# Linux-cpp-lisp/navigation-by-deja-vu

Hardware: AMD Instinct MI355X
Metric: view-comparisons/sec (sensor x library x headings) (higher is better)
Workload: dtype u8

## Files before the change

### include/dejavu.h

```cpp
#ifndef DEJAVU_H
#define DEJAVU_H

#include <stdint.h>

#ifdef __cplusplus
extern "C" {
#endif

typedef struct dv_ctx dv_ctx;

enum {
    DV_OK = 0,
    DV_ERR_INVALID = -1,
    DV_ERR_HIP = -2,
    DV_ERR_STATE = -3,
    DV_ERR_OOM = -4,
    DV_ERR_INDEX = -5
};

#define DV_MAX_HEADINGS 64
#define DV_MAX_HUE_PLANES 4

#define DV_STEP_FORCE_RESOLVE 1u
#define DV_STEP_WANT_SCENE    2u
// ... 201 lines not shown
int dv_timer_start(dv_ctx *ctx);
int dv_timer_stop(dv_ctx *ctx, float *elapsed_ms);
int dv_profile_kernel(dv_ctx *ctx, int enable);
int dv_profile_read(dv_ctx *ctx, double *total_ms, int64_t *n_launches);
int dv_workgroup_shape(dv_ctx *ctx, int n_headings, int *shape);
int dv_stream_read_gbps(dv_ctx *ctx, int64_t n_bytes, int iters, double *gbps);

int dv_range_push(const char *name);
int dv_range_pop(void);

int dv_patches_on_level(dv_ctx *ctx);

#define DV_FORM_MATRIX_CORES 1
#define DV_FORM_FP4 2
#define DV_FORM_FUSED_FINISH 4
int dv_scoring_form(dv_ctx *ctx);

const char *dv_version(void);

#ifdef __cplusplus
}
#endif
#endif
```

### navigation-by-deja-vu_amd/csrc/dejavu_hip.hip

```cpp
#include "dejavu_kernels.h"
#include "../../include/dejavu.h"

#include <algorithm>
#include <atomic>
#include <chrono>
#include <cmath>
#include <limits>
#include <cstdarg>
#include <cstddef>
#include <cstdint>
#include <cstdio>
#include <cstdlib>
#include <cstring>
#include <new>
#include <string>
#include <vector>

using namespace dv;

static_assert(sizeof(StepResultDev) == sizeof(dv_step_result) + sizeof(unsigned long long) &&
              offsetof(StepResultDev, check) == sizeof(dv_step_result), "device record = host record + check word");
static_assert(kMaxHeadings == DV_MAX_HEADINGS && kMaxHues == DV_MAX_HUE_PLANES, "header constants differ");
static_assert(kResSenseError == DV_RES_SENSE_ERROR, "header constants differ");

// ... 109 lines not shown
    size_t btile_bytes = 0;
    uint4* d_coef = nullptr;
    bool coef_ready = false;
    bool prep_dwords_ready = false;
    int bits_env = 1;
    int mfma_tiles_env = 0, mfma_chunk_env = 0;
    const int* int_hsconst = nullptr;
    const int* int_vconst = nullptr;
    bool fuse_request = false;
    bool epilogue_fused = false;
    bool fp4_ok = false;
    int fp4_env = 1;
    uint4* d_coef4 = nullptr;
    uint4* d_ctiles = nullptr;
    size_t ctile_bytes = 0;
    int vcode_env = 0;
    int last_form = 0;
    int fuse_env = 1;
    int lc_env = 1;
    int ht_env = 2;
    int ring_env = 0;
    int mixed_env = 1;
    int tune_all_env = 0;
    int fail_alloc_env = 0;
    int lib_allocs = 0;
    int fused_nb = 0;
    int group_pad_kb = -1;
    int allow_signed = 1;
    double* d_fam = nullptr;
    double* d_scene = nullptr;
    StepState* d_state = nullptr;
// ... 111 lines not shown
static void use_set(dv_ctx* c, int which);
static void diffuse_free(dv_ctx* c);
static void free_library(dv_ctx* c) {
    auto F = [](auto*& p) { if (p) { (void)hipFree(p); p = nullptr; } };
    use_set(c, 0);
    for (int j = 0; j < dv_ctx::kExtraSets; ++j) {
        dv_ctx::PassSet& a = c->extra[j];
        F(a.raw); F(a.coef); F(a.coef4); F(a.acc); F(a.bsum); F(a.ctmp); F(a.state); F(a.cand); F(a.cand_exact);
        a = dv_ctx::PassSet{};
    }
    c->n_extra = 0;
    F(c->d_tiles); F(c->d_raw_patches); F(c->d_prep); F(c->d_acc); F(c->d_one); F(c->d_fam); F(c->d_scene);
    F(c->d_part); F(c->d_pmax); F(c->d_record); F(c->d_keys); F(c->d_bsum); F(c->d_bsum2); F(c->d_ctmp);
    F(c->d_ftiles); F(c->d_fraw); F(c->d_fprep); F(c->d_fpart); F(c->d_fprep4); F(c->d_fvnorm); F(c->d_fpnorm); F(c->d_flower); F(c->d_fprepb);
    F(c->d_u8tiles); F(c->d_u8raw); F(c->d_u8prep); F(c->d_u8part); F(c->d_vnorm); F(c->d_pnorm);
    F(c->d_btiles); F(c->d_coef); F(c->d_coef4); F(c->d_ctiles); c->ctile_bytes = 0;
    c->pbits = PrepBits{};
    c->bits_ok = false; c->coef_ready = false; c->btile_bytes = 0;
    c->metric = 0;
    F(c->d_state); F(c->d_cand); F(c->d_cand_exact);
    if (c->h_result) { (void)hipHostFree(c->h_result); c->h_result = nullptr; c->d_result = nullptr; }
    if (c->h_scene) { (void)hipHostFree(c->h_scene); c->h_scene = nullptr; }
    F(c->d_scene_b);
    if (c->h_scene_b) { (void)hipHostFree(c->h_scene_b); c->h_scene_b = nullptr; }
    c->scene_b_cap = 0;
    c->have_lib = false;
    for (int i = 0; i < 4; ++i) c->tuned_shape[i] = 0;
    c->A = 0;
    c->step_pending = false;
}

// ... 208 lines not shown
    return DV_OK;
}

extern "C" int dv_synchronize(dv_ctx* c) {
    if (!c) return DV_ERR_INVALID;
    HIP_TRY(c, hipSetDevice(c->device));
    HIP_TRY(c, hipStreamSynchronize(c->stream));
    return DV_OK;
}

static long long group_stride(const dv_ctx* c, long long kb) {
    const long long pad = c->group_pad_kb >= 0 ? c->group_pad_kb : ((kb & 1) ? 0 : 1);
    return (kb + pad) * 64;
}

static int build_bit_planes(dv_ctx* c) {
    const LibCfg& g = c->cfg;
    c->bits_ok = false;
    c->fp4_ok = false;
    c->mixed = false;
    if (c->bits_env == 0 || c->metric != 0 || g.generic) return DV_OK;
    unsigned* d_presence = nullptr;
    uint32_t presence[(kMaxHues + 1) * 8];
    HIP_TRY(c, hipMalloc(&d_presence, sizeof presence));
    hipError_t e = hipMemsetAsync(d_presence, 0, sizeof presence, c->stream);
    if (e == hipSuccess) {
        hipLaunchKernelGGL(k_level_scan, dim3(2048), dim3(256), 0, c->stream, c->d_tiles, c->cfg, d_presence);
        e = hipGetLastError();
    }
    if (e == hipSuccess) e = hipMemcpyAsync(presence, d_presence, sizeof presence, hipMemcpyDeviceToHost, c->stream);
// ... 64 lines not shown
    for (int k = 0; k < kMaxBitPlanes; ++k)
        pb.tbl[k] = (unsigned)b.pl[k] | ((unsigned)b.lo[k] << 8) | ((unsigned)b.w[k] << 16) | ((unsigned)b.wfull[k] << 24);
    HIP_TRY(c, hipMemsetAsync(c->d_coef, 0, (size_t)2 * nkt * 8192, c->stream));
    if (c->fp4_ok) HIP_TRY(c, hipMemsetAsync(c->d_coef4, 0, (size_t)2 * nkt * 4096, c->stream));
    for (int bp = 0; bp < g.npl; ++bp) {
        pb.lmin[bp] = b.lmin[bp];
        for (int v = 0; v < 256; ++v) {
            const bool level = (presence[bp * 8 + (v >> 5)] >> (v & 31)) & 1u;
            if ((mixed && bp < g.nhs) || level || v <= (int)b.lmin[bp] || v >= (int)b.lmax[bp]) pb.ok[bp][v >> 5] |= 1u << (v & 31);
        }
    }
    c->pbits = pb;
    c->mixed = mixed;
    b.vcode = 0;
    b.GSC = b.GS;
    if (c->fp4_ok && five_levels) {
        const long long units = 4ll * b.NK[0] + 3ll * b.NK[1];
        long long kib = (units + 3) / 4;
        if (kib % 2 == 0) ++kib;
        b.GSC = (int)(kib * 4);
        if (hipMalloc(&c->d_ctiles, (size_t)G32 * b.GSC * 256) == hipSuccess) {
            b.vcode = 1;
            c->ctile_bytes = (size_t)G32 * units * 256;
        } else {
            (void)hipGetLastError();
            b.GSC = b.GS;
        }
    }
    b.nt = c->nt_env >= 0 ? c->nt_env : 1;
    c->bcfg = b;
    const long long total_t = G32 * nkt * 64;
    hipLaunchKernelGGL(k_bitpack, dim3((unsigned)((total_t + 255) / 256)), dim3(256), 0, c->stream, c->d_tiles, c->d_btiles, c->cfg, b);
    HIP_TRY(c, hipGetLastError());
    if (b.vcode) {
        hipLaunchKernelGGL(k_bitpack_code, dim3((unsigned)((total_t + 255) / 256)), dim3(256), 0, c->stream, c->d_btiles,
                           reinterpret_cast<unsigned*>(c->d_ctiles), c->cfg, b);
        HIP_TRY(c, hipGetLastError());
    }
    HIP_TRY(c, hipStreamSynchronize(c->stream));
    c->bits_ok = true;
    c->coef_ready = false;
    return DV_OK;
}

static const unsigned* offlevel_word(const dv_ctx* c) {
    return c->fp4_ok ? &c->d_acc[c->acc_parity].off : c->d_one;
}
static int enqueue_bit_prep(dv_ctx* c, bool force = false) {
    (void)force;
// ... 1101 lines not shown
    return word == 0 ? 1 : 0;
}

extern "C" int dv_patches_on_level(dv_ctx* c) {
    if (!c) return DV_ERR_INVALID;
    if (!c->have_lib || !c->bits_ok || !c->fp4_ok) return fail(c, DV_ERR_STATE, "this library has no fp4 form");
    if (!c->coef_ready) return fail(c, DV_ERR_STATE, "no coefficient image of the resident patches yet");
    return read_on_level(c);
}

extern "C" int dv_scoring_form(dv_ctx* c) {
    if (!c) return DV_ERR_INVALID;
    if (!(c->last_form & DV_FORM_FP4)) return c->last_form;
    const int on_level = read_on_level(c);
    if (on_level < 0) return on_level;
    return on_level ? c->last_form : c->last_form & ~DV_FORM_FP4;
}

extern "C" int dv_clear_library(dv_ctx* c) {
    if (!c) return DV_ERR_INVALID;
    HIP_TRY(c, hipSetDevice(c->device));
    HIP_TRY(c, hipStreamSynchronize(c->stream));
    free_library(c);
    return DV_OK;
}

extern "C" int dv_get_library_info(const dv_ctx* c, dv_lib_info* o) {
    if (!c || !o) return DV_ERR_INVALID;
    if (!c->have_lib) return DV_ERR_STATE;
    memset(o, 0, sizeof *o);
    o->n_views = c->cfg.F;
// ... 6 lines not shown
    o->signed_saturation = c->cfg.signed_s;
    o->has_value_plane = c->cfg.hasv;
    o->tile_bytes = (int64_t)c->tile_bytes;
    o->chem_weight = c->cfg.cw;
    o->delta = c->delta;
    for (int k = 0; k < kMaxHues; ++k) o->hues[k] = c->cfg.hues[k];
    o->n_hues = 0;
    if (c->cfg.has_hs && !c->cfg.generic) o->n_hues = c->cfg.signed_s ? 2 : c->cfg.nhs;
    o->weight_lo = c->cfg.hasv ? 0.0 : 1.0;
    o->weight_hi = c->cfg.has_hs ? 1.0 : 0.0;
    o->has_bit_planes = c->bits_ok ? 1 : 0;
    o->fp4_form = (c->bits_ok && c->fp4_ok) ? 1 : 0;
    o->bit_planes_hs = c->bits_ok ? c->bcfg.T[0] : 0;
    o->bit_planes_v = c->bits_ok ? c->bcfg.T[1] : 0;
    o->bit_tile_bytes = c->bits_ok ? (int64_t)c->btile_bytes : 0;
    o->code_tile_bytes = (c->bits_ok && c->bcfg.vcode) ? (int64_t)c->ctile_bytes : 0;
    o->mixed_layout = (c->bits_ok && c->mixed) ? 1 : 0;
    return DV_OK;
}

extern "C" int dv_read_planes(dv_ctx* c, int64_t v0, int64_t n, uint8_t* out) {
    if (!c || !out) return DV_ERR_INVALID;
    if (!c->have_lib) return fail(c, DV_ERR_STATE, "no library set");
    if (v0 < 0 || n < 1 || v0 + n > c->cfg.F) return fail(c, DV_ERR_INVALID, "view range [%lld, %lld) outside the library", (long long)v0, (long long)(v0 + n));
    HIP_TRY(c, hipSetDevice(c->device));
    const long long total = n * c->cfg.npl * (long long)c->cfg.P;
    unsigned char* d = nullptr;
    HIP_TRY(c, hipMalloc(&d, (size_t)total));
    hipLaunchKernelGGL(k_read_planes, dim3((unsigned)((total + 255) / 256)), dim3(256), 0, c->stream, c->d_tiles, d, c->cfg,
                       (long long)v0, (long long)n);
    hipError_t e = hipGetLastError();
// ... 158 lines not shown

static FuseArgs fuse_args(const dv_ctx* c) {
    FuseArgs fz{};
    fz.wts = wts_ptr(c);
    fz.hsconst = c->d_acc[c->acc_parity].bhs;
    fz.vconst = c->d_acc[c->acc_parity].bv;
    fz.bsum = c->d_bsum;
    fz.ctmp = c->d_ctmp;
    fz.st = c->d_state;
    fz.A_real = c->A;
    fz.A_agent = c->A_agent;
    fz.delta = c->delta;
    return fz;
}

enum class Body { Ring, Ring2, RingA, RingB, Lc, LcShort, LcCode, LcReg, Lc2Tiles, Lc2TilesCode, Lc22, Count };

struct BodyShape { int SK8, RD8, SK4, RD4, TILES, SKL, RDL; bool LCODE; int HT; };
constexpr BodyShape kBodyShapes[] = {
     {4, 2, 2, 4, 1, 0, 3, false, 1},
     {1, 3, 2, 3, 2, 0, 3, false, 1},
     {4, 2, 2, 6, 1, 0, 3, false, 1},
     {4, 2, 4, 3, 1, 0, 3, false, 1},
     {4, 2, 2, 4, 1, 4, 3, false, 1},
     {4, 2, 2, 4, 1, 2, 5, false, 1},
     {4, 2, 2, 4, 1, 4, 3, true, 1},
     {4, 2, 2, 4, 1, kLregStage, 3, false, 1},
     {4, 2, 2, 4, 1, 4, 3, false, 2},
     {4, 2, 2, 4, 1, 4, 3, true, 2},
     {4, 2, 0, 0, 1, 2, 3, false, 2},
};
static_assert(sizeof kBodyShapes / sizeof kBodyShapes[0] == (size_t)Body::Count, "one shape per body");
constexpr BodyShape body_shape(Body b) { return kBodyShapes[(int)b]; }

template <Body B, bool FUSE>
constexpr auto body_kernel() {
    constexpr BodyShape s = body_shape(B);
    if constexpr (B == Body::Lc22) return &k_sad_lc22<s.SKL, s.RDL>;
    else return &k_sad_mfma_dual<s.SK8, s.RD8, s.SK4, s.RD4, s.TILES, FUSE, s.SKL, s.RDL, s.LCODE, s.HT>;
}

constexpr int body_view_groups(Body b) { return b == Body::Lc22 ? 8 : 8 * body_shape(b).TILES / body_shape(b).HT; }
// ... 17 lines not shown

template <Body B, bool FUSE>
static void launch_body(dv_ctx* c, int nchunk, int has_hs) {
    constexpr BodyShape s = body_shape(B);
    constexpr int lds = body_lds_bytes<B, FUSE>();
    static_assert(body_lds_bytes<B, true>() <= 160 * 1024, "LDS");
    constexpr auto kernel = body_kernel<B, FUSE>();
    static const hipError_t attr_set = hipFuncSetAttribute((const void*)kernel, hipFuncAttributeMaxDynamicSharedMemorySize, lds);
    (void)attr_set;
    const long long n_gq = item_groups(c->cfg.Fpad / 32, body_view_groups(B));
    const long long items = n_gq * nchunk;
    const unsigned grid = (unsigned)(items < 256 ? items : 256);
    const int nkt = c->bcfg.NK[0] + c->bcfg.NK[1];
    FuseArgs fz{};
    if (FUSE) { fz = fuse_args(c); fz.nb = (int)grid; }
    for (int a_off = 0; a_off < c->APAD; a_off += 32 * s.HT) {
        const uint4* coef = c->d_coef + (size_t)(a_off / 32) * nkt * 512;
        const uint4* coef4 = c->fp4_ok ? c->d_coef4 + (size_t)(a_off / 32) * nkt * 256 : nullptr;
        if constexpr (B == Body::Lc22) {
            hipLaunchKernelGGL(kernel, dim3(grid), dim3(512), lds, c->stream, c->d_btiles, coef, coef4, offlevel_word(c), c->cfg, c->bcfg,
                               c->APAD, a_off, has_hs, fz, (int)n_gq);
        } else {
            hipLaunchKernelGGL(kernel, dim3(grid), dim3(512), lds, c->stream, c->d_btiles, c->bcfg.vcode ? c->d_ctiles : c->d_btiles, coef,
                               coef4, offlevel_word(c), reinterpret_cast<int*>(c->d_part), c->cfg, c->bcfg, nchunk, c->APAD, a_off, has_hs,
                               fz, (int)n_gq);
        }
    }
    if (FUSE) { c->epilogue_fused = true; c->fused_nb = (int)grid; }
}

static bool shared_accumulator_fits(const dv_ctx* c, bool with_bit0) {
    if (!c->fp4_ok || c->bcfg.vcode || c->mixed) return false;
    for (int seg = 0; seg < 2; ++seg) {
        int w = 0;
        for (int bit = 1; bit < 4; ++bit) {
            const int wb = c->bcfg.wacc[seg][bit];
            if (wb && w && wb != w) return false;
            if (wb) w = wb;
        }
        if (with_bit0 && seg == 0 && c->bcfg.wacc[0][0] && w && c->bcfg.wacc[0][0] != w) return false;
    }
    return true;
}
static bool lc22_fits(const dv_ctx* c) {
    return shared_accumulator_fits(c, true) && (long long)c->bcfg.NK[0] * 256 <= 32767;
}
static bool lreg_fits(const dv_ctx* c) {
    return shared_accumulator_fits(c, false) && c->bcfg.NK[0] % kLregStage == 0;
}

struct MfmaPlan { Body body; int nchunk; bool fuses; };
static MfmaPlan mfma_plan(dv_ctx* c, int apad, bool fuse_request) {
    const long long G32 = c->cfg.Fpad / 32;
    const bool may_fuse = fuse_request && c->fuse_env && !c->mfma_chunk_env;
    const bool use_lc = c->lc_env != 0 && c->fp4_ok && !c->mfma_tiles_env;
    Body body;
    if (use_lc) {
        const bool two_tiles = apad == 64 && c->ht_env == 2;
        if (two_tiles && may_fuse && c->lc22_env && lc22_fits(c) && item_groups(G32, 8) >= 160) body = Body::Lc22;
        else if (two_tiles) body = c->bcfg.vcode ? Body::Lc2TilesCode : Body::Lc2Tiles;
        else if (c->bcfg.vcode) body = Body::LcCode;
        else body = c->lc_env == 2 ? Body::LcShort : Body::Lc;
    } else {
        const int tiles = c->mfma_tiles_env ? c->mfma_tiles_env : (G32 >= 16ll * 320 ? 2 : 1);
        body = tiles == 2 ? Body::Ring2 : (c->ring_env == 1 ? Body::RingA : (c->ring_env == 2 ? Body::RingB : Body::Ring));
        if (body == Body::Ring2 && !c->mfma_tiles_env) {
            static const bool spills[2] = {kernel_uses_scratch((const void*)body_kernel<Body::Ring2, false>()),
                                           kernel_uses_scratch((const void*)body_kernel<Body::Ring2, true>())};
            const bool will_fuse = may_fuse && item_groups(G32, body_view_groups(Body::Ring2)) >= 160;
            if (spills[will_fuse ? 1 : 0]) body = c->ring_env == 1 ? Body::RingA : (c->ring_env == 2 ? Body::RingB : Body::Ring);
        }
    }
    const long long GQ = item_groups(G32, body_view_groups(body));
    int nchunk = 1;
    if (c->mfma_chunk_env) {
        nchunk = c->mfma_chunk_env;
    } else if (GQ < 160) {
        nchunk = (int)((256 + GQ - 1) / GQ);
    }
    const int nk_min = c->bcfg.NK[1] > 0 ? (c->bcfg.NK[0] > 0 && c->bcfg.NK[0] < c->bcfg.NK[1] ? c->bcfg.NK[0] : c->bcfg.NK[1]) : c->bcfg.NK[0];
    while (nchunk > 1 && nk_min / nchunk < 4) --nchunk;
    if (nchunk > c->nchunk_cap) nchunk = c->nchunk_cap;
    if (nchunk < 1 || c->mixed) nchunk = 1;
    if (body == Body::Lc && nchunk == 1 && c->lreg_env && lreg_fits(c)) body = Body::LcReg;
    return {body, nchunk, fuse_request && c->fuse_env && nchunk == 1};
}

static bool batch_pass_fuses(dv_ctx* c, int apad) {
    if (c->metric != 0 || c->exact || c->cfg.generic || !c->bits_ok || c->mixed) return false;
    const int cls = apad_class(apad);
    const int shape = c->shape_env ? c->shape_env : c->tuned_shape[cls];
    if (shape != 6) return false;
    return mfma_plan(c, apad, true).fuses;
}

template <Body B>
static void launch_planned(dv_ctx* c, const MfmaPlan& p, int has_hs) {
    if constexpr (B != Body::Lc22) {
        if (!p.fuses) return launch_body<B, false>(c, p.nchunk, has_hs);
    }
    launch_body<B, true>(c, p.nchunk, has_hs);
}

static void launch_mfma(dv_ctx* c, int has_hs) {
    const MfmaPlan p = mfma_plan(c, c->APAD, c->fuse_request);
    c->nchunk = p.nchunk;
    switch (p.body) {
        case Body::Ring: return launch_planned<Body::Ring>(c, p, has_hs);
        case Body::Ring2: return launch_planned<Body::Ring2>(c, p, has_hs);
        case Body::RingA: return launch_planned<Body::RingA>(c, p, has_hs);
        case Body::RingB: return launch_planned<Body::RingB>(c, p, has_hs);
        case Body::Lc: return launch_planned<Body::Lc>(c, p, has_hs);
        case Body::LcShort: return launch_planned<Body::LcShort>(c, p, has_hs);
        case Body::LcCode: return launch_planned<Body::LcCode>(c, p, has_hs);
        case Body::LcReg: return launch_planned<Body::LcReg>(c, p, has_hs);
        case Body::Lc2Tiles: return launch_planned<Body::Lc2Tiles>(c, p, has_hs);
        case Body::Lc2TilesCode: return launch_planned<Body::Lc2TilesCode>(c, p, has_hs);
        case Body::Lc22: return launch_planned<Body::Lc22>(c, p, has_hs);
        case Body::Count: break;
    }
}

static int launch_int_scoring(dv_ctx* c, hipEvent_t after_tiles, int* n_partial, bool with_combine = true) {
    const LibCfg& g = c->cfg;
    int has_hs_sum, has_v_sum = g.hasv;
    c->int_hsconst = c->d_acc[c->acc_parity].hs;
    c->int_vconst = nullptr;
    c->epilogue_fused = false;
    c->last_form = 0;
    if (needs_prep_dwords(c)) { const int rc = ensure_prep_dwords(c); if (rc) return rc; }
// ... 6 lines not shown
            HIP_TRY(c, hipGetLastError());
            c->hs_bytes_pass = true;
            const int keep = c->force_shape;
            c->force_shape = c->APAD >= 16 ? 2 : 1;
            switch (g.nhs) {
                case 1: launch_tiles_apad<1, 0>(c); break;
                case 2: launch_tiles_apad<2, 0>(c); break;
                case 3: launch_tiles_apad<3, 0>(c); break;
                default: launch_tiles_apad<4, 0>(c); break;
            }
            c->force_shape = keep;
            c->hs_bytes_pass = false;
            c->nchunk = 1;
        } else
        launch_mfma(c, has_hs_sum);
        c->last_form = DV_FORM_MATRIX_CORES | (c->fp4_ok ? DV_FORM_FP4 : 0) | (c->epilogue_fused ? DV_FORM_FUSED_FINISH : 0);
        c->int_hsconst = c->mixed ? c->d_acc[c->acc_parity].hs : c->d_acc[c->acc_parity].bhs;
        c->int_vconst = c->d_acc[c->acc_parity].bv;
    } else if (g.generic) {
        has_hs_sum = 1;
        if (g.hasv) launch_generic_apad<1, 1>(c); else launch_generic_apad<1, 0>(c);
    } else {
        has_hs_sum = g.nhs > 0 ? 1 : 0;
        switch (g.nhs * 2 + g.hasv) {
            case 1: launch_tiles_apad<0, 1>(c); break;
            case 2: launch_tiles_apad<1, 0>(c); break;
            case 3: launch_tiles_apad<1, 1>(c); break;
            case 4: launch_tiles_apad<2, 0>(c); break;
            case 5: launch_tiles_apad<2, 1>(c); break;
            case 6: launch_tiles_apad<3, 0>(c); break;
            case 7: launch_tiles_apad<3, 1>(c); break;
// ... 998 lines not shown
```

### navigation-by-deja-vu_amd/csrc/dejavu_kernels.h

```cpp
#pragma once
#include <hip/hip_runtime.h>
#include <stdint.h>
#include <type_traits>

#pragma clang fp contract(off)

namespace dv {

#ifdef DEJAVU_STAMPS
#ifdef DEJAVU_EXP_FIN
#define DV_EXP_FIN_ON 1
#else
#define DV_EXP_FIN_ON 0
#endif
__device__ unsigned long long g_dv_stamps[256 * 8];
#define DV_STAMP(i) do { if (threadIdx.x == 0) { g_dv_stamps[(blockIdx.x & 255) * 8 + (i)] = __builtin_amdgcn_s_memrealtime(); \
    if (((i) == 1 || (i) == 2) && !DV_EXP_FIN_ON) g_dv_stamps[(blockIdx.x & 255) * 8 + 5 + (i)] = __builtin_amdgcn_s_memtime(); } } while (0)
#else
#define DV_STAMP(i) do { } while (0)
#endif

constexpr int kMaxHeadings = 64;
constexpr int kMaxHues = 4;
constexpr int kCandCap = 4096;
// ... 3609 lines not shown
        }
    }
    }
    if constexpr (FUSE) {
#pragma unroll
        for (int h = 0; h < HT; ++h)
            if (a_off + 32 * h < fz.A_real) fused_block_end(scratch0 + h * 64, fz, c, a_off + 32 * h);
    }
    DV_STAMP(5);
}

constexpr int kLregStage = 8;
template <int SK, int RD>
constexpr int lreg_ring_bytes() { return RD * SK * 4 * 1024; }

template <int SK, int RD, bool FUSE>
__device__ __forceinline__ void
sad_lc_fp4_lreg(const uint4* __restrict__ btiles, const uint4* __restrict__ coef4, int* __restrict__ part, const LibCfg& c, const BitCfg& b,
                int apad_total, int a_off, int has_hs_sum, const FuseArgs& fz, int n_gq) {
    extern __shared__ uint4 lds_ring[];
    constexpr int TL = 2;
    constexpr int NW = 8, NC = 4;
    constexpr int KCOEF = 4;
    constexpr int SLOTB = SK * KCOEF * 1024;
    constexpr int PER = SK;
    constexpr int RING = RD * SLOTB;
    static_assert(PER * (RD - 1) < 64 && SK % 2 == 0 && RD >= 3, "ring shape");
    const int lane = threadIdx.x & 63;
    const int wave = __builtin_amdgcn_readfirstlane(threadIdx.x >> 6);
    const bool loader = wave >= NC;
    const long long G32 = c.Fpad / 32, GQ = n_gq;
    const int NKT = b.NK[0] + b.NK[1];
    const int nst = (NKT + SK - 1) / SK;
    const int NK0 = b.NK[0];
    const long long gbytes = (long long)b.GS * 1024;
    const unsigned lds_base = (unsigned)(unsigned long long)(lds_ptr_t)lds_ring;
    unsigned long long* scratch0 = reinterpret_cast<unsigned long long*>(reinterpret_cast<unsigned char*>(lds_ring) + RING);
    const unsigned char* lib_bytes = reinterpret_cast<const unsigned char*>(btiles);
    DV_STAMP(0);
    if constexpr (FUSE) fused_block_begin(scratch0, true);
    const long long n_mine = GQ > (long long)blockIdx.x ? (GQ - blockIdx.x + gridDim.x - 1) / gridDim.x : 0;

    if (loader) {
        const int lw = wave - NC;
        long long li = 0;
        int lst = 0, lslot = 0;
        auto issue_stage = [&]() {
            const unsigned slot = lds_base + (unsigned)lslot * (unsigned)SLOTB;
            const int kb = lst * SK;
            const uint4* hot = coef4 + lw * 64 + lane;
// ... 42 lines not shown
                const long long g = g0 + wave * TL + t;
                cp[t] = lib_bytes + (g < g1 ? g : g0) * gbytes + lane * 16;
            }
        };
        v4u_t xr[SK][TL];
        auto load_row = [&](int kk) {
            int k = lkb + kk;
            k = k < NKT ? k : NKT - 1;
#pragma unroll
            for (int t = 0; t < TL; ++t) xr[kk][t] = __builtin_nontemporal_load(reinterpret_cast<const v4u_t*>(cp[t] + (long long)k * 1024));
        };
        auto cursor_next = [&]() {
            lkb += SK;
            if (lkb >= nst * SK) { lkb = 0; ++lj; cursor_item(); }
        };
        if (n_mine > 0) {
            cursor_item();
#pragma unroll
            for (int kk = 0; kk < SK; ++kk) load_row(kk);
            cursor_next();
        }
        for (long long j = 0; j < n_mine; ++j) {
            const long long item = blockIdx.x + j * gridDim.x;
            const long long g0 = (item * G32) / GQ, g1 = ((item + 1) * G32) / GQ;
            long long gidx[TL];
            bool live[TL];
#pragma unroll
            for (int t = 0; t < TL; ++t) {
                const long long g = g0 + wave * TL + t;
                live[t] = g < g1;
                gidx[t] = live[t] ? g : g0;
            }
            int tot_hs[TL][16], tot_v[TL][16];
#pragma unroll
            for (int t = 0; t < TL; ++t)
// ... 80 lines not shown
                            for (int s = 0; s < 4; ++s) {
                                const v4u_t& av = a[kk & 1][s];
                                const v8i_t ao = v8i_t{(int)av.x, (int)av.y, (int)av.z, (int)av.w, 0, 0, 0, 0};
#pragma unroll
                                for (int t = 0; t < TL; ++t) {
                                    const v8i_t bv = v8i_t{(int)bo[t][s][0], (int)bo[t][s][1], (int)bo[t][s][2], (int)bo[t][s][3], 0, 0, 0, 0};
                                    if constexpr (FUSE) acc[t][s ? 1 : 0] = __builtin_amdgcn_mfma_scale_f32_32x32x64_f8f6f4(bv, ao, acc[t][s ? 1 : 0], 4, 4, 0, 0, 0, 0);
                                    else acc[t][s ? 1 : 0] = __builtin_amdgcn_mfma_scale_f32_32x32x64_f8f6f4(ao, bv, acc[t][s ? 1 : 0], 4, 4, 0, 0, 0, 0);
                                }
                            }
                        });
                        cursor_next();
                        cslot = nslot;
                    }
                };
                const int nst0 = has_hs_sum ? (NK0 / SK < nst ? NK0 / SK : nst) : 0;
                const int hs_end = (has_hs_sum && !(c.hasv && b.NK[1] > 0)) ? nst : nst0;
                run_stages(0, hs_end);
                if (hs_end > 0 && hs_end < nst) {
                    flush(tot_hs, 0);
                    if constexpr (!FUSE) store_sums(tot_hs, 0);
                    clear();
                }
                run_stages(hs_end, nst);
                if (hs_end < nst) flush(tot_v, 1);
                else flush(tot_hs, 0);
                if constexpr (!FUSE) {
                    if (has_hs_sum && !(hs_end > 0 && hs_end < nst)) store_sums(tot_hs, 0);
                    if (c.hasv) store_sums(tot_v, 1);
                }
            }
            if (j == 0) DV_STAMP(2);
            if constexpr (FUSE) {
                if (j == 0) DV_STAMP(3);
                auto of_hs = [&](int t, int r) -> int { return tot_hs[t][r]; };
                auto of_v = [&](int t, int r) -> int { return tot_v[t][r]; };
                fused_finish<TL, NW, true>(of_hs, of_v, gidx, live, scratch0, c, fz, a_off, has_hs_sum, j, lane, wave, (int)(j & 1), NC, hconst);
                if (j == 0) DV_STAMP(4);
            }
        }
    }
    if constexpr (FUSE) {
        if (a_off < fz.A_real) fused_block_end(scratch0, fz, c, a_off);
    }
    DV_STAMP(5);
}

template <int SK, int RD>
constexpr int lc22_ring_bytes() { return RD * SK * 16 * 1024; }
constexpr int kLc22ParkBytes = 4 * 64 * 64 * 2;

template <int SK, int RD>
__device__ __forceinline__ void
sad_lc22_fp4(const uint4* __restrict__ ftiles, const uint4* __restrict__ coef4, const LibCfg& c, const BitCfg& b, int apad_total, int a_off,
             int has_hs_sum, const FuseArgs& fz, int n_gq) {
// ... 298 lines not shown
        if (h > 0 && a_off + 32 * h >= apad_total) break;
        sad_ring_i8<4, 1, 2, true>(btiles, coef + (long long)h * NKT * 512, nullptr, c, b, 1, apad_total, a_off + 32 * h, has_hs_sum, fz, n_gq);
    }
}

template <int SK8, int RD8, int SK4, int RD4, int TILES, bool FUSE, int SKL, int RDL, bool LCODE, int HT>
__global__ void __launch_bounds__(512, 2)
k_sad_mfma_dual(const uint4* __restrict__ btiles, const uint4* __restrict__ ftiles, const uint4* __restrict__ coef, const uint4* __restrict__ coef4,
                const unsigned* __restrict__ offlevel, int* __restrict__ part, LibCfg c, BitCfg b, int nchunk, int apad_total, int a_off,
                int has_hs_sum, FuseArgs fz, int n_gq) {
    const bool fp4 = __builtin_amdgcn_readfirstlane(*offlevel) == 0u;
    if constexpr (SKL > 0) {
        static_assert(TILES == 1, "the loader / consumer body cuts the library into ranges of 8 / HT view groups; the other bodies must agree");
        if (fp4 && nchunk == 1) {
            if constexpr (SKL == kLregStage) {
                static_assert(HT == 1 && !LCODE, "sad_lc_fp4_lreg: one heading tile, thermometer rows");
                sad_lc_fp4_lreg<SKL, RDL, FUSE>(btiles, coef4, part, c, b, apad_total, a_off, has_hs_sum, fz, n_gq);
            } else {
                sad_lc_fp4<SKL, RDL, FUSE, LCODE, HT>(ftiles, coef4, part, c, b, apad_total, a_off, has_hs_sum, fz, n_gq);
            }
            return;
        }
    }
    const int NKT = b.NK[0] + b.NK[1];
#pragma unroll 1
    for (int h = 0; h < HT; ++h) {
        if (h > 0 && a_off + 32 * h >= apad_total) break;
        if (fp4) sad_ring_fp4<SK4, TILES, RD4, FUSE>(btiles, coef4 + (long long)h * NKT * 256, part, c, b, nchunk, apad_total, a_off + 32 * h, has_hs_sum, fz, n_gq);
        else sad_ring_i8<SK8, TILES, RD8, FUSE>(btiles, coef + (long long)h * NKT * 512, part, c, b, nchunk, apad_total, a_off + 32 * h, has_hs_sum, fz, n_gq);
    }
}

// ... 25 lines not shown
```

### navigation-by-deja-vu_amd/navsim_amd/engine.py

```python
import ctypes

import numpy as np

from . import _native as N


def agent_weights(chem_weights, n):
    if chem_weights is None:
        return None
    w = np.ascontiguousarray(chem_weights, dtype=np.float64).reshape(-1)
    if w.shape[0] != n:
        raise ValueError("chem_weights holds %d weights for %d agents" % (w.shape[0], n))
    return w


class BatchResults(object):
    _DTYPE = np.dtype(N.StepResult)

    def __init__(self, raw, n, A, scene=None):
        self._raw, self.n, self.A = raw, n, A
        self.scene_familiarity = scene
        rec = np.frombuffer(raw, dtype=self._DTYPE, count=n)
        self.records = rec
        self.best_idex, self.best_view, self.step_familiarity = rec["best_heading"], rec["best_view"], rec["best_fam"]
# ... 595 lines not shown
    def path_coverage(self, n):
        out = np.empty(int(n), dtype=np.uint8)
        self._check(self._lib.dv_path_coverage(self._ctx, N.u8ptr(out), int(n)), "dv_path_coverage")
        return out.astype(bool)

    def patches_on_level(self):
        rc = self._lib.dv_patches_on_level(self._ctx)
        if rc < 0:
            self._check(rc, "dv_patches_on_level")
        return bool(rc)

    def scoring_form(self):
        rc = self._lib.dv_scoring_form(self._ctx)
        if rc < 0:
            self._check(rc, "dv_scoring_form")
        return dict(matrix_cores=bool(rc & 1), fp4=bool(rc & 2), fused_finish=bool(rc & 4))

    def path_reset(self):
        self._check(self._lib.dv_path_reset(self._ctx), "dv_path_reset")

    def path_slots(self, n_slots):
        self._check(self._lib.dv_path_slots(self._ctx, int(n_slots)), "dv_path_slots")

    def path_error_batch(self, slots, xs, ys, reach):
        slots = np.ascontiguousarray(slots, dtype=np.int32)
        xs = np.ascontiguousarray(xs, dtype=np.float64)
        ys = np.ascontiguousarray(ys, dtype=np.float64)
        out = np.empty(len(slots), dtype=np.float64)
        self._check(self._lib.dv_path_error_batch(self._ctx, slots.ctypes.data_as(ctypes.POINTER(ctypes.c_int32)), N.f64ptr(xs), N.f64ptr(ys),
                                                  len(slots), float(reach), N.f64ptr(out)), "dv_path_error_batch")
        return out
# ... 15 lines not shown
```

Measured before the change: 15.61 billion.

## Add code-tile variant of register-staged fp4 scoring kernel to cut library bytes

Adds a LcRegCode body in which the register-staged fp4 MFMA kernel reads compact 3-bit code tiles instead of 4-bit thermometer bit planes. Thermometer rows are rebuilt in registers with shifts and masks, and library reads use nontemporal global loads with immediate offsets. Code tiles are now built by default whenever the planner would choose this body. The aim is to cut HBM traffic per view comparison at the cost of extra ALU decode work, more complex vmcnt wait accounting, and extra memory for the code tiles.

New measurement: 16.93 billion, median of 6. 8.5% higher.

```diff
diff --git a/include/dejavu.h b/include/dejavu.h
--- a/include/dejavu.h
+++ b/include/dejavu.h
@@ -239,6 +239,7 @@
 #define DV_FORM_MATRIX_CORES 1
 #define DV_FORM_FP4 2
 #define DV_FORM_FUSED_FINISH 4
+#define DV_FORM_CODES 8
 int dv_scoring_form(dv_ctx *ctx);
 
 const char *dv_version(void);
diff --git a/navigation-by-deja-vu_amd/csrc/dejavu_hip.hip b/navigation-by-deja-vu_amd/csrc/dejavu_hip.hip
--- a/navigation-by-deja-vu_amd/csrc/dejavu_hip.hip
+++ b/navigation-by-deja-vu_amd/csrc/dejavu_hip.hip
@@ -147,7 +147,9 @@
     uint4* d_coef4 = nullptr;
     uint4* d_ctiles = nullptr;
     size_t ctile_bytes = 0;
-    int vcode_env = 0;
+    int vcode_env = -1;
+    bool code_all = false;
+    bool last_codes = false;
     int last_form = 0;
     int fuse_env = 1;
     int lc_env = 1;
@@ -289,7 +291,7 @@
     F(c->d_part); F(c->d_pmax); F(c->d_record); F(c->d_keys); F(c->d_bsum); F(c->d_bsum2); F(c->d_ctmp);
     F(c->d_ftiles); F(c->d_fraw); F(c->d_fprep); F(c->d_fpart); F(c->d_fprep4); F(c->d_fvnorm); F(c->d_fpnorm); F(c->d_flower); F(c->d_fprepb);
     F(c->d_u8tiles); F(c->d_u8raw); F(c->d_u8prep); F(c->d_u8part); F(c->d_vnorm); F(c->d_pnorm);
-    F(c->d_btiles); F(c->d_coef); F(c->d_coef4); F(c->d_ctiles); c->ctile_bytes = 0;
+    F(c->d_btiles); F(c->d_coef); F(c->d_coef4); F(c->d_ctiles); c->ctile_bytes = 0; c->code_all = false;
     c->pbits = PrepBits{};
     c->bits_ok = false; c->coef_ready = false; c->btile_bytes = 0;
     c->metric = 0;
@@ -528,6 +530,7 @@
     return (kb + pad) * 64;
 }
 
+static bool plan_reads_codes(dv_ctx* c);
 static int build_bit_planes(dv_ctx* c) {
     const LibCfg& g = c->cfg;
     c->bits_ok = false;
@@ -622,25 +625,27 @@
     c->mixed = mixed;
     b.vcode = 0;
     b.GSC = b.GS;
-    if (c->fp4_ok && five_levels) {
+    b.nt = c->nt_env >= 0 ? c->nt_env : 1;
+    c->bcfg = b;
+    if (c->fp4_ok && five_levels && (c->vcode_env == 1 || plan_reads_codes(c))) {
         const long long units = 4ll * b.NK[0] + 3ll * b.NK[1];
         long long kib = (units + 3) / 4;
         if (kib % 2 == 0) ++kib;
         b.GSC = (int)(kib * 4);
         if (hipMalloc(&c->d_ctiles, (size_t)G32 * b.GSC * 256) == hipSuccess) {
-            b.vcode = 1;
+            c->code_all = c->vcode_env == 1;
             c->ctile_bytes = (size_t)G32 * units * 256;
         } else {
             (void)hipGetLastError();
+            c->d_ctiles = nullptr;
             b.GSC = b.GS;
         }
     }
-    b.nt = c->nt_env >= 0 ? c->nt_env : 1;
     c->bcfg = b;
     const long long total_t = G32 * nkt * 64;
     hipLaunchKernelGGL(k_bitpack, dim3((unsigned)((total_t + 255) / 256)), dim3(256), 0, c->stream, c->d_tiles, c->d_btiles, c->cfg, b);
     HIP_TRY(c, hipGetLastError());
-    if (b.vcode) {
+    if (c->d_ctiles) {
         hipLaunchKernelGGL(k_bitpack_code, dim3((unsigned)((total_t + 255) / 256)), dim3(256), 0, c->stream, c->d_btiles,
                            reinterpret_cast<unsigned*>(c->d_ctiles), c->cfg, b);
         HIP_TRY(c, hipGetLastError());
@@ -1772,7 +1777,7 @@
     if (!(c->last_form & DV_FORM_FP4)) return c->last_form;
     const int on_level = read_on_level(c);
     if (on_level < 0) return on_level;
-    return on_level ? c->last_form : c->last_form & ~DV_FORM_FP4;
+    return on_level ? c->last_form : c->last_form & ~(DV_FORM_FP4 | DV_FORM_CODES);
 }
 
 extern "C" int dv_clear_library(dv_ctx* c) {
@@ -1809,7 +1814,7 @@
     o->bit_planes_hs = c->bits_ok ? c->bcfg.T[0] : 0;
     o->bit_planes_v = c->bits_ok ? c->bcfg.T[1] : 0;
     o->bit_tile_bytes = c->bits_ok ? (int64_t)c->btile_bytes : 0;
-    o->code_tile_bytes = (c->bits_ok && c->bcfg.vcode) ? (int64_t)c->ctile_bytes : 0;
+    o->code_tile_bytes = (c->bits_ok && c->d_ctiles) ? (int64_t)c->ctile_bytes : 0;
     o->mixed_layout = (c->bits_ok && c->mixed) ? 1 : 0;
     return DV_OK;
 }
@@ -1998,7 +2003,7 @@
     return fz;
 }
 
-enum class Body { Ring, Ring2, RingA, RingB, Lc, LcShort, LcCode, LcReg, Lc2Tiles, Lc2TilesCode, Lc22, Count };
+enum class Body { Ring, Ring2, RingA, RingB, Lc, LcShort, LcCode, LcReg, LcRegCode, Lc2Tiles, Lc2TilesCode, Lc22, Count };
 
 struct BodyShape { int SK8, RD8, SK4, RD4, TILES, SKL, RDL; bool LCODE; int HT; };
 constexpr BodyShape kBodyShapes[] = {
@@ -2010,6 +2015,7 @@
      {4, 2, 2, 4, 1, 2, 5, false, 1},
      {4, 2, 2, 4, 1, 4, 3, true, 1},
      {4, 2, 2, 4, 1, kLregStage, 3, false, 1},
+     {4, 2, 2, 4, 1, kLregStage, 3, true, 1},
      {4, 2, 2, 4, 1, 4, 3, false, 2},
      {4, 2, 2, 4, 1, 4, 3, true, 2},
      {4, 2, 0, 0, 1, 2, 3, false, 2},
@@ -2057,6 +2063,10 @@
     const int nkt = c->bcfg.NK[0] + c->bcfg.NK[1];
     FuseArgs fz{};
     if (FUSE) { fz = fuse_args(c); fz.nb = (int)grid; }
+    BitCfg bcfg = c->bcfg;
+    bcfg.vcode = s.LCODE ? 1 : 0;
+    const uint4* ftiles = s.LCODE ? c->d_ctiles : c->d_btiles;
+    c->last_codes = s.LCODE && nchunk == 1;
     for (int a_off = 0; a_off < c->APAD; a_off += 32 * s.HT) {
         const uint4* coef = c->d_coef + (size_t)(a_off / 32) * nkt * 512;
         const uint4* coef4 = c->fp4_ok ? c->d_coef4 + (size_t)(a_off / 32) * nkt * 256 : nullptr;
@@ -2064,8 +2074,8 @@
             hipLaunchKernelGGL(kernel, dim3(grid), dim3(512), lds, c->stream, c->d_btiles, coef, coef4, offlevel_word(c), c->cfg, c->bcfg,
                                c->APAD, a_off, has_hs, fz, (int)n_gq);
         } else {
-            hipLaunchKernelGGL(kernel, dim3(grid), dim3(512), lds, c->stream, c->d_btiles, c->bcfg.vcode ? c->d_ctiles : c->d_btiles, coef,
-                               coef4, offlevel_word(c), reinterpret_cast<int*>(c->d_part), c->cfg, c->bcfg, nchunk, c->APAD, a_off, has_hs,
+            hipLaunchKernelGGL(kernel, dim3(grid), dim3(512), lds, c->stream, c->d_btiles, ftiles, coef,
+                               coef4, offlevel_word(c), reinterpret_cast<int*>(c->d_part), c->cfg, bcfg, nchunk, c->APAD, a_off, has_hs,
                                fz, (int)n_gq);
         }
     }
@@ -2073,7 +2083,7 @@
 }
 
 static bool shared_accumulator_fits(const dv_ctx* c, bool with_bit0) {
-    if (!c->fp4_ok || c->bcfg.vcode || c->mixed) return false;
+    if (!c->fp4_ok || c->code_all || c->mixed) return false;
     for (int seg = 0; seg < 2; ++seg) {
         int w = 0;
         for (int bit = 1; bit < 4; ++bit) {
@@ -2091,9 +2101,12 @@
 static bool lreg_fits(const dv_ctx* c) {
     return shared_accumulator_fits(c, false) && c->bcfg.NK[0] % kLregStage == 0;
 }
+static bool lreg_code_fits(const dv_ctx* c) {
+    return lreg_fits(c) && c->cfg.hasv && c->bcfg.T[1] == 4 && c->bcfg.NK[1] > 0 && c->bcfg.NK[1] % kLregStage == 0;
+}
 
 struct MfmaPlan { Body body; int nchunk; bool fuses; };
-static MfmaPlan mfma_plan(dv_ctx* c, int apad, bool fuse_request) {
+static MfmaPlan mfma_plan(dv_ctx* c, int apad, bool fuse_request, bool assume_code_tiles) {
     const long long G32 = c->cfg.Fpad / 32;
     const bool may_fuse = fuse_request && c->fuse_env && !c->mfma_chunk_env;
     const bool use_lc = c->lc_env != 0 && c->fp4_ok && !c->mfma_tiles_env;
@@ -2101,8 +2114,8 @@
     if (use_lc) {
         const bool two_tiles = apad == 64 && c->ht_env == 2;
         if (two_tiles && may_fuse && c->lc22_env && lc22_fits(c) && item_groups(G32, 8) >= 160) body = Body::Lc22;
-        else if (two_tiles) body = c->bcfg.vcode ? Body::Lc2TilesCode : Body::Lc2Tiles;
-        else if (c->bcfg.vcode) body = Body::LcCode;
+        else if (two_tiles) body = c->code_all ? Body::Lc2TilesCode : Body::Lc2Tiles;
+        else if (c->code_all) body = Body::LcCode;
         else body = c->lc_env == 2 ? Body::LcShort : Body::Lc;
     } else {
         const int tiles = c->mfma_tiles_env ? c->mfma_tiles_env : (G32 >= 16ll * 320 ? 2 : 1);
@@ -2126,7 +2139,12 @@
     if (nchunk > c->nchunk_cap) nchunk = c->nchunk_cap;
     if (nchunk < 1 || c->mixed) nchunk = 1;
     if (body == Body::Lc && nchunk == 1 && c->lreg_env && lreg_fits(c)) body = Body::LcReg;
+    if (body == Body::LcReg && (c->d_ctiles || assume_code_tiles) && lreg_code_fits(c)) body = Body::LcRegCode;
     return {body, nchunk, fuse_request && c->fuse_env && nchunk == 1};
+}
+
+static bool plan_reads_codes(dv_ctx* c) {
+    return mfma_plan(c, 32, true, true).body == Body::LcRegCode;
 }
 
 static bool batch_pass_fuses(dv_ctx* c, int apad) {
@@ -2134,7 +2152,7 @@
     const int cls = apad_class(apad);
     const int shape = c->shape_env ? c->shape_env : c->tuned_shape[cls];
     if (shape != 6) return false;
-    return mfma_plan(c, apad, true).fuses;
+    return mfma_plan(c, apad, true, false).fuses;
 }
 
 template <Body B>
@@ -2146,7 +2164,7 @@
 }
 
 static void launch_mfma(dv_ctx* c, int has_hs) {
-    const MfmaPlan p = mfma_plan(c, c->APAD, c->fuse_request);
+    const MfmaPlan p = mfma_plan(c, c->APAD, c->fuse_request, false);
     c->nchunk = p.nchunk;
     switch (p.body) {
         case Body::Ring: return launch_planned<Body::Ring>(c, p, has_hs);
@@ -2157,6 +2175,7 @@
         case Body::LcShort: return launch_planned<Body::LcShort>(c, p, has_hs);
         case Body::LcCode: return launch_planned<Body::LcCode>(c, p, has_hs);
         case Body::LcReg: return launch_planned<Body::LcReg>(c, p, has_hs);
+        case Body::LcRegCode: return launch_planned<Body::LcRegCode>(c, p, has_hs);
         case Body::Lc2Tiles: return launch_planned<Body::Lc2Tiles>(c, p, has_hs);
         case Body::Lc2TilesCode: return launch_planned<Body::Lc2TilesCode>(c, p, has_hs);
         case Body::Lc22: return launch_planned<Body::Lc22>(c, p, has_hs);
@@ -2193,7 +2212,8 @@
             c->nchunk = 1;
         } else
         launch_mfma(c, has_hs_sum);
-        c->last_form = DV_FORM_MATRIX_CORES | (c->fp4_ok ? DV_FORM_FP4 : 0) | (c->epilogue_fused ? DV_FORM_FUSED_FINISH : 0);
+        c->last_form = DV_FORM_MATRIX_CORES | (c->fp4_ok ? DV_FORM_FP4 : 0) | (c->epilogue_fused ? DV_FORM_FUSED_FINISH : 0) |
+                       (c->fp4_ok && c->last_codes ? DV_FORM_CODES : 0);
         c->int_hsconst = c->mixed ? c->d_acc[c->acc_parity].hs : c->d_acc[c->acc_parity].bhs;
         c->int_vconst = c->d_acc[c->acc_parity].bv;
     } else if (g.generic) {
diff --git a/navigation-by-deja-vu_amd/csrc/dejavu_kernels.h b/navigation-by-deja-vu_amd/csrc/dejavu_kernels.h
--- a/navigation-by-deja-vu_amd/csrc/dejavu_kernels.h
+++ b/navigation-by-deja-vu_amd/csrc/dejavu_kernels.h
@@ -3647,7 +3647,13 @@
 template <int SK, int RD>
 constexpr int lreg_ring_bytes() { return RD * SK * 4 * 1024; }
 
-template <int SK, int RD, bool FUSE>
+template <int OFF>
+__device__ __forceinline__ void lib_load16_nt(v4u_t& d, unsigned voff, unsigned long long base) {
+    static_assert(OFF >= 0 && OFF < 4096, "immediate offset");
+    asm volatile("global_load_dwordx4 %0, %1, %2 offset:%3 nt" : "+v"(d) : "v"(voff), "s"(base), "n"(OFF) : "memory");
+}
+
+template <int SK, int RD, bool FUSE, bool CODE>
 __device__ __forceinline__ void
 sad_lc_fp4_lreg(const uint4* __restrict__ btiles, const uint4* __restrict__ coef4, int* __restrict__ part, const LibCfg& c, const BitCfg& b,
                 int apad_total, int a_off, int has_hs_sum, const FuseArgs& fz, int n_gq) {
@@ -3666,7 +3672,7 @@
     const int NKT = b.NK[0] + b.NK[1];
     const int nst = (NKT + SK - 1) / SK;
     const int NK0 = b.NK[0];
-    const long long gbytes = (long long)b.GS * 1024;
+    const long long gbytes = CODE ? (long long)b.GSC * 256 : (long long)b.GS * 1024;
     const unsigned lds_base = (unsigned)(unsigned long long)(lds_ptr_t)lds_ring;
     unsigned long long* scratch0 = reinterpret_cast<unsigned long long*>(reinterpret_cast<unsigned char*>(lds_ring) + RING);
     const unsigned char* lib_bytes = reinterpret_cast<const unsigned char*>(btiles);
@@ -3739,11 +3745,47 @@
             lkb += SK;
             if (lkb >= nst * SK) { lkb = 0; ++lj; cursor_item(); }
         };
+        const int n_sat = has_hs_sum ? NK0 / SK : 0;
+        const unsigned voff = (unsigned)lane * 16u;
+        unsigned long long cbase[TL] = {0, 0}, cstage[TL] = {0, 0};
+        auto cursor_stage_code = [&]() {
+            const int vk = lkb - n_sat * SK;
+            const unsigned off = (unsigned)lkb * 1024u - (unsigned)(vk > 0 ? vk : 0) * 256u;
+#pragma unroll
+            for (int t = 0; t < TL; ++t) cstage[t] = cbase[t] + off;
+        };
+        auto cursor_item_code = [&]() {
+            const long long item = blockIdx.x + (lj < n_mine ? lj : 0) * gridDim.x;
+            const long long g0 = (item * G32) / GQ, g1 = ((item + 1) * G32) / GQ;
+#pragma unroll
+            for (int t = 0; t < TL; ++t) {
+                const long long g = g0 + wave * TL + t;
+                cbase[t] = (unsigned long long)(lib_bytes + (g < g1 ? g : g0) * gbytes);
+            }
+            cursor_stage_code();
+        };
+        auto load_piece = [&](auto ec) {
+            constexpr int e = decltype(ec)::value;
+#pragma unroll
+            for (int t = 0; t < TL; ++t) lib_load16_nt<(e & 3) * 1024>(xr[e][t], voff, cstage[t] + (e >> 2) * 4096u);
+        };
+        auto cursor_next_code = [&]() {
+            lkb += SK;
+            if (lkb >= nst * SK) { lkb = 0; ++lj; cursor_item_code(); }
+            else cursor_stage_code();
+        };
         if (n_mine > 0) {
-            cursor_item();
-#pragma unroll
-            for (int kk = 0; kk < SK; ++kk) load_row(kk);
-            cursor_next();
+            if constexpr (CODE) {
+                cursor_item_code();
+                static_for<6>([&](auto ec) { load_piece(ec); });
+                if (n_sat > 0) { load_piece(IntC<6>{}); load_piece(IntC<7>{}); }
+                cursor_next_code();
+            } else {
+                cursor_item();
+#pragma unroll
+                for (int kk = 0; kk < SK; ++kk) load_row(kk);
+                cursor_next();
+            }
         }
         for (long long j = 0; j < n_mine; ++j) {
             const long long item = blockIdx.x + j * gridDim.x;
@@ -3854,8 +3896,100 @@
                         cslot = nslot;
                     }
                 };
+                auto run_code = [&](int s0, int s1, auto ckc, auto lkc) {
+                    constexpr int CK = decltype(ckc)::value, LK = decltype(lkc)::value;
+                    for (int st = s0; st < s1; ++st) {
+                        const int nslot = cslot + 1 == RD ? 0 : cslot + 1;
+                        static_for<SK>([&](auto kc) {
+                            constexpr int kk = decltype(kc)::value;
+                            if constexpr (kk + 1 < SK) {
+                                fetch(cslot, IntC<kk + 1>{});
+                                lds_wait<4>();
+                            } else {
+                                lds_wait<0>();
+                                if (st + 1 < nst) {
+                                    __builtin_amdgcn_s_barrier();
+                                    fetch(nslot, IntC<0>{});
+                                }
+                            }
+#pragma unroll
+                            for (int s = 0; s < 4; ++s) lds_tie(a[kk & 1][s]);
+                            constexpr unsigned m = 0x22222222u;
+                            constexpr int h3 = 3 * (kk / 4), q = kk % 4;
+                            constexpr int newest = CK ? h3 + (q < 2 ? q : 2) : kk;
+                            constexpr int sent = CK ? kk - (kk + 3) / 4 : (LK == 0 || kk < 6 ? kk : 6);
+                            wait_vmcnt_le<TL * ((CK ? 6 : 8) - 1 - newest + sent)>();
+                            unsigned bo[TL][4][4];
+                            if constexpr (CK == 0) {
+#pragma unroll
+                                for (int t = 0; t < TL; ++t) lds_tie(xr[kk][t]);
+#pragma unroll
+                                for (int t = 0; t < TL; ++t) {
+                                    const unsigned x[4] = {xr[kk][t].x, xr[kk][t].y, xr[kk][t].z, xr[kk][t].w};
+#pragma unroll
+                                    for (int d = 0; d < 4; ++d) {
+                                        bo[t][0][d] = (x[d] << 1) & m;
+                                        bo[t][1][d] = x[d] & m;
+                                        bo[t][2][d] = (x[d] >> 1) & m;
+                                        bo[t][3][d] = (x[d] >> 2) & m;
+                                    }
+                                }
+                                if constexpr (LK == 0 || kk < 6) load_piece(kc);
+                            } else {
+#pragma unroll
+                                for (int t = 0; t < TL; ++t) {
+                                    if constexpr (q < 2) lds_tie(xr[h3][t]);
+                                    if constexpr (q == 1 || q == 2) lds_tie(xr[h3 + 1][t]);
+                                    if constexpr (q >= 2) lds_tie(xr[h3 + 2][t]);
+                                }
+#pragma unroll
+                                for (int t = 0; t < TL; ++t) {
+                                    unsigned x[4];
+                                    if constexpr (q == 0) { x[0] = xr[h3][t].x; x[1] = xr[h3][t].y; x[2] = xr[h3][t].z; }
+                                    else if constexpr (q == 1) { x[0] = xr[h3][t].w; x[1] = xr[h3 + 1][t].x; x[2] = xr[h3 + 1][t].y; }
+                                    else if constexpr (q == 2) { x[0] = xr[h3 + 1][t].z; x[1] = xr[h3 + 1][t].w; x[2] = xr[h3 + 2][t].x; }
+                                    else { x[0] = xr[h3 + 2][t].y; x[1] = xr[h3 + 2][t].z; x[2] = xr[h3 + 2][t].w; }
+                                    x[3] = ((x[0] >> 3) & 0x11111111u) | ((x[1] >> 2) & 0x22222222u) | ((x[2] >> 1) & 0x44444444u);
+#pragma unroll
+                                    for (int d = 0; d < 4; ++d) {
+                                        bo[t][0][d] = ((x[d] << 1) | x[d]) & m;
+                                        bo[t][1][d] = x[d] & m;
+                                        bo[t][2][d] = (x[d] >> 1) & m;
+                                        bo[t][3][d] = (x[d] << 1) & (x[d] >> 1) & m;
+                                    }
+                                }
+                                if constexpr (q > 0) load_piece(IntC<kk - 1 - kk / 4>{});
+                                if constexpr (LK == 0 && kk == SK - 1) { load_piece(IntC<6>{}); load_piece(IntC<7>{}); }
+                            }
+#pragma unroll
+                            for (int s = 0; s < 4; ++s) {
+                                const v4u_t& av = a[kk & 1][s];
+                                const v8i_t ao = v8i_t{(int)av.x, (int)av.y, (int)av.z, (int)av.w, 0, 0, 0, 0};
+#pragma unroll
+                                for (int t = 0; t < TL; ++t) {
+                                    const v8i_t bv = v8i_t{(int)bo[t][s][0], (int)bo[t][s][1], (int)bo[t][s][2], (int)bo[t][s][3], 0, 0, 0, 0};
+                                    if constexpr (FUSE) acc[t][s ? 1 : 0] = __builtin_amdgcn_mfma_scale_f32_32x32x64_f8f6f4(bv, ao, acc[t][s ? 1 : 0], 4, 4, 0, 0, 0, 0);
+                                    else acc[t][s ? 1 : 0] = __builtin_amdgcn_mfma_scale_f32_32x32x64_f8f6f4(ao, bv, acc[t][s ? 1 : 0], 4, 4, 0, 0, 0, 0);
+                                }
+                            }
+                        });
+                        cursor_next_code();
+                        cslot = nslot;
+                    }
+                };
                 const int nst0 = has_hs_sum ? (NK0 / SK < nst ? NK0 / SK : nst) : 0;
                 const int hs_end = (has_hs_sum && !(c.hasv && b.NK[1] > 0)) ? nst : nst0;
+                if constexpr (CODE) {
+                    if (hs_end > 0) {
+                        run_code(0, hs_end - 1, IntC<0>{}, IntC<0>{});
+                        run_code(hs_end - 1, hs_end, IntC<0>{}, IntC<1>{});
+                        flush(tot_hs, 0);
+                        if constexpr (!FUSE) store_sums(tot_hs, 0);
+                        clear();
+                    }
+                    run_code(hs_end, hs_end > 0 ? nst - 1 : nst, IntC<1>{}, IntC<1>{});
+                    if (hs_end > 0) run_code(nst - 1, nst, IntC<1>{}, IntC<0>{});
+                } else {
                 run_stages(0, hs_end);
                 if (hs_end > 0 && hs_end < nst) {
                     flush(tot_hs, 0);
@@ -3863,6 +3997,7 @@
                     clear();
                 }
                 run_stages(hs_end, nst);
+                }
                 if (hs_end < nst) flush(tot_v, 1);
                 else flush(tot_hs, 0);
                 if constexpr (!FUSE) {
@@ -3879,6 +4014,7 @@
                 if (j == 0) DV_STAMP(4);
             }
         }
+        if constexpr (CODE) wait_vmcnt_le<0>();
     }
     if constexpr (FUSE) {
         if (a_off < fz.A_real) fused_block_end(scratch0, fz, c, a_off);
@@ -4207,8 +4343,8 @@
         static_assert(TILES == 1, "the loader / consumer body cuts the library into ranges of 8 / HT view groups; the other bodies must agree");
         if (fp4 && nchunk == 1) {
             if constexpr (SKL == kLregStage) {
-                static_assert(HT == 1 && !LCODE, "sad_lc_fp4_lreg: one heading tile, thermometer rows");
-                sad_lc_fp4_lreg<SKL, RDL, FUSE>(btiles, coef4, part, c, b, apad_total, a_off, has_hs_sum, fz, n_gq);
+                static_assert(HT == 1, "sad_lc_fp4_lreg: one heading tile");
+                sad_lc_fp4_lreg<SKL, RDL, FUSE, LCODE>(LCODE ? ftiles : btiles, coef4, part, c, b, apad_total, a_off, has_hs_sum, fz, n_gq);
             } else {
                 sad_lc_fp4<SKL, RDL, FUSE, LCODE, HT>(ftiles, coef4, part, c, b, apad_total, a_off, has_hs_sum, fz, n_gq);
             }
diff --git a/navigation-by-deja-vu_amd/navsim_amd/engine.py b/navigation-by-deja-vu_amd/navsim_amd/engine.py
--- a/navigation-by-deja-vu_amd/navsim_amd/engine.py
+++ b/navigation-by-deja-vu_amd/navsim_amd/engine.py
@@ -633,7 +633,7 @@
         rc = self._lib.dv_scoring_form(self._ctx)
         if rc < 0:
             self._check(rc, "dv_scoring_form")
-        return dict(matrix_cores=bool(rc & 1), fp4=bool(rc & 2), fused_finish=bool(rc & 4))
+        return dict(matrix_cores=bool(rc & 1), fp4=bool(rc & 2), fused_finish=bool(rc & 4), codes=bool(rc & 8))
 
     def path_reset(self):
         self._check(self._lib.dv_path_reset(self._ctx), "dv_path_reset")
```
